# guxm2021/SVT_SpeechBrain

Hardware: AMD Instinct MI355X
Metric: 10s@16kHz clips/sec encoder+CTC forward, wav2vec2-base, 1/2/4/8 MI355X (higher is better)
Workload: dtype bf16; 1 GPU; wav2vec2-base audio-only AMT forward (encoder + 20-way head + frame decode), 32 x 10 s @16 kHz mono clips per GPU; global_batch=32, per_gpu_batch=32, samples_per_clip=160000, frames_per_clip=499, parallelism=clips sharded over 1 rank(s), streams=2, inputs=resident in HBM

## Files before the change

svt_speechbrain_amd/csrc/gemm_dma.hip:

```cpp
#include "common.h"
#include <map>
#include <mutex>
#include <utility>

namespace svt {
namespace {

__device__ __forceinline__ float gelu_erf(float x) { return gelu_fast(x); }
__device__ __forceinline__ float apply_act(float v, int act) {
  if (act == ACT_GELU) return gelu_erf(v);
  if (act == ACT_RELU) return v > 0.f ? v : 0.f;
  return v;
}

typedef const void __attribute__((address_space(1)))* gptr_t;
typedef void __attribute__((address_space(3)))* lptr_t;

template <int N> __device__ __forceinline__ void wait_vm() { asm volatile("s_waitcnt vmcnt(%0)" ::"n"(N) : "memory"); }

struct BiasRegs { float v[8]; };
template <bool OUT32>
__device__ __forceinline__ BiasRegs load_bias_regs(const GemmArgs& p, const float* bias, int lane, int wn, int n0) {
  BiasRegs b;
#pragma unroll
// ... 881 lines not shown
      long long* o = p.trace + 65536 + ((long)blockIdx.x * 8 + wave) * 32;
#pragma unroll
      for (int i = 0; i < 5; ++i) o[i] = sst[i];
      o[9] = nk; o[10] = gs; o[11] = STQ;
    }
  }
#undef X3S_S
#undef X3S_COMMIT
#undef X3S_LOAD
#undef X3S_MMA
#undef X3S_VARS
#undef X3S_END
  wait_vm<0>();
  __syncthreads();
  const float* bias = p.bias ? p.bias + (long)z2 * p.bias_z2 : nullptr;
  float* patch = (float*)lds + wave * (16 * 68);
  if constexpr (DBG == 3) {
#pragma unroll
    for (int i = 0; i < NB; ++i) asm volatile("" ::"v"(acc[i][0]), "v"(acc[i][1]));
    return;
  }
#pragma unroll
  for (int g = 0; g < NBS; ++g) {
    const BiasRegs br = load_bias_regs<true>(p, bias, lane, g, n0);
    epilogue_block<2, 64, true>(p, acc[4 * g][0], acc[4 * g + 1][0], acc[4 * g + 2][0], acc[4 * g + 3][0], 0, patch, lane, wave, g, m0, n0, czoff, br);
    epilogue_block<2, 64, true>(p, acc[4 * g][1], acc[4 * g + 1][1], acc[4 * g + 2][1], acc[4 * g + 3][1], 1, patch, lane, wave, g, m0, n0, czoff, br);
  }
}

template <bool F16>
__global__ void split_pack_kernel(const float* __restrict__ w, long n_rows, int K, unsigned short* __restrict__ out) {
  const long i = (long)blockIdx.x * blockDim.x + threadIdx.x;
  const long per_row = K / 8;
  if (i >= n_rows * per_row) return;
  const long n = i / per_row;
  const int k0 = (int)(i % per_row) * 8;
  const float* src = w + n * K + k0;
  unsigned short h[8], l[8];
#pragma unroll
  for (int j = 0; j < 8; ++j) {
    const float x = src[j];
    if constexpr (F16) {
      const _Float16 a = (_Float16)x, b = (_Float16)(x - (float)a);
      h[j] = __builtin_bit_cast(unsigned short, a);
      l[j] = __builtin_bit_cast(unsigned short, b);
    } else {
      const bf16_t a = (bf16_t)x, b = (bf16_t)(x - (float)a);
      h[j] = __builtin_bit_cast(unsigned short, a);
      l[j] = __builtin_bit_cast(unsigned short, b);
    }
  }
  unsigned short* dst = out + n * (2L * K) + (long)(k0 / 32) * 64 + (k0 % 32);
#pragma unroll
  for (int j = 0; j < 8; ++j) { dst[j] = h[j]; dst[32 + j] = l[j]; }
}

template <int BM>
int launch_pers(const GemmArgs& a, hipStream_t s) {
  const int tiles_m = (a.M + BM - 1) / BM, tiles_n = (a.N + 255) / 256;
  const int ntiles = tiles_m * tiles_n;
  int nblk = ntiles < 256 ? ((ntiles + 7) / 8) * 8 : 256;
  const size_t lds_bytes = 5 * 32768;
  if (int r_ = ensure_dyn_lds((const void*)gemm_pers_kernel<BM>, (int)lds_bytes)) return r_;
  const double flops = 2.0 * a.M * (double)a.N * a.K;
  const double bytes = ((double)a.M * a.K + (double)a.N * a.K) * 2 + (double)a.M * a.N * (a.out_f32 ? 4 : 2);
  prof_begin(s);
  hipLaunchKernelGGL((gemm_pers_kernel<BM>), dim3(nblk), dim3(512), lds_bytes, s, a, tiles_n, ntiles);
  prof_end(s, flops, bytes, 0);
  SVT_LAUNCH_CHECK();
  return 0;
}

template <int BM, bool GEN = false, int NBW = 4>
int launch_pp8(const GemmArgs& a, hipStream_t s) {
  const int tiles_m = (a.M + BM - 1) / BM, tiles_n = (a.N + 64 * NBW - 1) / (64 * NBW);
  dim3 grid(tiles_m * tiles_n, a.nz, 1);
  const size_t lds_bytes = 5 * 32768;
  if (int r_ = ensure_dyn_lds((const void*)gemm_pp8_kernel<BM, GEN, NBW>, (int)lds_bytes)) return r_;
  const double flops = 2.0 * a.M * (double)a.N * a.K * a.nz;
  const double bytes = ((double)a.M * a.K + (double)a.N * a.K) * 2 * a.nz + (double)a.M * a.N * a.nz * (a.out_f32 ? 4 : 2);
  prof_begin(s);
  hipLaunchKernelGGL((gemm_pp8_kernel<BM, GEN, NBW>), grid, dim3(512), lds_bytes, s, a);
  prof_end(s, flops, bytes, 0);
  SVT_LAUNCH_CHECK();
  return 0;
}

}

namespace {
struct SplitW { void* packed; int N, K, kind; };
std::map<const void*, SplitW> g_split_w;
std::mutex g_split_mu;
}

int split_weights_register(const void* w_f32, long n_rows, int K, int kind, hipStream_t s) {
  if (kind != 2 && kind != 3) return 0;
  if (K % 32 || n_rows < 1) return 0;
  void* packed = nullptr;
  {
    std::lock_guard<std::mutex> lk(g_split_mu);
    auto it = g_split_w.find(w_f32);
    if (it != g_split_w.end() && it->second.N == (int)n_rows && it->second.K == K) packed = it->second.packed;
  }
  const bool reused = packed != nullptr;
  if (reused) SVT_HIP(hipDeviceSynchronize());
  if (!reused)
    if (int r = dev_alloc(&packed, (size_t)n_rows * K * 4)) return r;
  const long pieces = n_rows * (K / 8);
  if (kind == 3) hipLaunchKernelGGL((split_pack_kernel<true>), dim3((unsigned)((pieces + 255) / 256)), dim3(256), 0, s, (const float*)w_f32, n_rows, K, (unsigned short*)packed);
  else hipLaunchKernelGGL((split_pack_kernel<false>), dim3((unsigned)((pieces + 255) / 256)), dim3(256), 0, s, (const float*)w_f32, n_rows, K, (unsigned short*)packed);
  SVT_LAUNCH_CHECK();
  std::lock_guard<std::mutex> lk(g_split_mu);
  auto it = g_split_w.find(w_f32);
  if (it != g_split_w.end() && !reused) dev_free(it->second.packed);
  g_split_w[w_f32] = SplitW{packed, (int)n_rows, K, kind};
  return 0;
}
void split_weights_forget(const void* w_f32) {
  std::lock_guard<std::mutex> lk(g_split_mu);
  auto it = g_split_w.find(w_f32);
  if (it == g_split_w.end()) return;
  dev_free(it->second.packed);
  g_split_w.erase(it);
}
int g_gemm_walk = -1;
int g_conv_kperm = 1;
int g_gemm_persist_wgs = 256;
int gemm_walk_pm(const GemmArgs& a, int bm) {
  if (g_gemm_walk >= 0) return g_gemm_walk;
  const int tiles_n = a.N / 256, tiles_m = (a.M + bm - 1) / bm;
  const double w_bytes = (double)a.N * a.K * 2.0;
  if (tiles_n < 8 || tiles_m < 16 || w_bytes <= 4.0 * 1024 * 1024) return 0;
  return 8;
}
int g_x3_pairs = 1;
int launch_gemm_x3(int kind, const GemmArgs& a, hipStream_t s) {
  if (a.a_pairs) {
    if (!gemm_x3q_eligible(a) || a.ldw != a.K) { set_error("gemm: pair-row operand outside the contract of gemm_x3q_kernel"); return -1; }
    const void* packed = nullptr;
    {
      std::lock_guard<std::mutex> lk(g_split_mu);
      auto it = g_split_w.upper_bound(a.W);
      if (it != g_split_w.begin()) {
        --it;
        const size_t off = (const char*)a.W - (const char*)it->first;
        if (it->second.kind == kind && it->second.K == a.K && off % ((size_t)a.K * 4) == 0 && off / ((size_t)a.K * 4) + a.N <= (size_t)it->second.N)
          packed = (const char*)it->second.packed + off;
      }
    }
    if (!packed) { set_error("gemm: pair-row product against a weight matrix that was not registered as split"); return -1; }
    const int cands[3] = {256, 192, 128};
    const int slab_cost[3] = {167, 137, 105};
    long best_cost = -1;
    int best = 256;
    for (int i = 0; i < 3; ++i) {
      const long blocks = (long)((a.M + cands[i] - 1) / cands[i]) * (a.N / 256);
      const long cost = ((blocks + 255) / 256) * slab_cost[i];
      if (best_cost < 0 || cost < best_cost) { best_cost = cost; best = cands[i]; }
    }
    if (g_gemm_force_bm == 256 || g_gemm_force_bm == 192 || g_gemm_force_bm == 128) best = g_gemm_force_bm;
    GemmArgs g = a;
    g.planes_f16 = kind == 3;
    const double flops = 2.0 * a.M * (double)a.N * a.K;
    const double bytes = ((double)a.M * a.K + (double)a.N * a.K + (double)a.M * a.N) * 4;
    prof_begin(s);
    if (g_gemm_p1x && g.K >= 96) { if (int r_ = launch_gemm_p1x(kind, g, packed, best, s)) return r_; }
    else if (int r_ = launch_gemm_x3q(kind, g, packed, best, s)) return r_;
    prof_end(s, flops, bytes, 0);
    return 0;
  }
  const bool batched = a.nz > 1;
  if (a.gen || a.nz < 1 || a.K % 32 || a.N < 128 || a.M < 128 || !a.c_vec || a.ldw != a.K || a.alpha != 1.f || (a.a_rstride & 3) ||
      (a.a_bstride & 3) || ((uintptr_t)a.A & 15))
    return 1;
  if (!batched && (a.w_z1 || a.w_z2 || a.a_z1 || a.a_z2 || a.c_z1 || a.c_z2)) return 1;
  if (batched && (a.planes || a.resid || a.nz2 < 1 || a.nz % a.nz2 || (a.a_z1 & 3) || (a.a_z2 & 3) || (a.c_z1 & 3) || (a.c_z2 & 3) || (a.bias_z2 & 3) ||
                  a.w_z1 % a.K || a.w_z2 % a.K || a.nz > 65535))
    return 1;
  const void* packed = nullptr;
  {
    std::lock_guard<std::mutex> lk(g_split_mu);
    auto it = g_split_w.upper_bound(a.W);
    if (it == g_split_w.begin()) return 1;
    --it;
    const char* base = (const char*)it->first;
    const size_t off = (const char*)a.W - base;
    if (it->second.kind != kind || it->second.K != a.K || off % ((size_t)a.K * 4) != 0) return 1;
    const size_t row = off / ((size_t)a.K * 4);
    const size_t last_z_row = batched ? ((size_t)(a.nz / a.nz2 - 1) * a.w_z1 + (size_t)(a.nz2 - 1) * a.w_z2) / (size_t)a.K : 0;
    if (row + last_z_row + a.N > (size_t)it->second.N) return 1;
    packed = (const char*)it->second.packed + row * (size_t)a.K * 4;
  }
  {
    const unsigned long clips = 255 / (unsigned long)(a.a_rpb > 0 ? a.a_rpb : 1) + 1;
    const unsigned long bs = (unsigned long)(a.a_bstride > 0 ? a.a_bstride : 0), rs = (unsigned long)(a.a_rstride > 0 ? a.a_rstride : 0);
    if (a.a_bstride < 0 || a.a_rstride <= 0 || (clips * bs + 256ul * rs + (unsigned long)a.K) * 4 >= 0xF0000000ul ||
        (unsigned long)a.N * a.K * 4 >= 0xF0000000ul)
      return 1;
  }
  const size_t lds_bytes = 5 * 32768;
  GemmArgs g = a;
  g.out_f32 = 1;
  g.planes_f16 = kind == 3;
  if (g_gemm_dbg == 9 && a.resid) {
    g.trace = (long long*)a.resid;
    g.resid = nullptr;
    g.stamp_ends = g_stamp_ends;
  }
  const double flops = 2.0 * a.M * (double)a.N * a.K * a.nz;
  const double bytes = ((double)a.M * a.K + (double)a.N * a.K + (double)a.M * a.N) * 4 * a.nz;
  const long tm = (a.M + 255) / 256;
  const long t256 = tm * ((a.N + 255) / 256), t192 = tm * ((a.N + 191) / 192);
  auto rounds = [](long t) { return (t + 255) / 256; };
  const bool narrow = a.N % 192 == 0 && rounds(t192) * 3 < rounds(t256) * 4;
  prof_begin(s);
  const bool x3p_ok = !batched && gemm_x3p_eligible(g) && g_gemm_variant != 30 && g_gemm_variant != 31 && g_gemm_variant != 32 && g_gemm_variant != 33;
  if (x3p_ok && (g_gemm_variant == 34 || (a.act == ACT_GELU && t256 > 256) || t256 >= 1024)) {
    g.dbg = g_gemm_dbg == 9 ? 0 : g_gemm_dbg;
    if (int r_ = launch_gemm_x3p(kind, g, packed, s)) return r_;
#ifdef SVT_DIAG
  } else if (g.trace && kind == 3 && g.stamp_ends >= 1 && g.stamp_ends <= 4) {
#define SVT_X3S_STAMP(NBS_, D_)                                                                                    \
  {                                                                                                                 \
    if (int r_ = ensure_dyn_lds((const void*)gemm_x3s_kernel<true, NBS_, D_>, (int)lds_bytes)) return r_;           \
    hipLaunchKernelGGL((gemm_x3s_kernel<true, NBS_, D_>), dim3((unsigned)(narrow ? t192 : t256)), dim3(512), lds_bytes, s, g, packed); \
  }
    if (narrow) {
      if (g.stamp_ends == 1) SVT_X3S_STAMP(3, 11) else if (g.stamp_ends == 2) SVT_X3S_STAMP(3, 12)
      else if (g.stamp_ends == 3) SVT_X3S_STAMP(3, 13) else SVT_X3S_STAMP(3, 14)
    } else {
      if (g.stamp_ends == 1) SVT_X3S_STAMP(4, 11) else if (g.stamp_ends == 2) SVT_X3S_STAMP(4, 12)
      else if (g.stamp_ends == 3) SVT_X3S_STAMP(4, 13) else SVT_X3S_STAMP(4, 14)
    }
#undef SVT_X3S_STAMP
  } else if ((g_gemm_variant == 31 || g_gemm_variant == 33) && kind == 3) {
    if (g_gemm_variant == 31) {
      if (int r_ = ensure_dyn_lds((const void*)gemm_x3s_kernel<true, 4, 1>, (int)lds_bytes)) return r_;
      hipLaunchKernelGGL((gemm_x3s_kernel<true, 4, 1>), dim3((unsigned)t256), dim3(512), lds_bytes, s, g, packed);
    } else {
      if (int r_ = ensure_dyn_lds((const void*)gemm_x3s_kernel<true, 4, 3>, (int)lds_bytes)) return r_;
      hipLaunchKernelGGL((gemm_x3s_kernel<true, 4, 3>), dim3((unsigned)t256), dim3(512), lds_bytes, s, g, packed);
    }
#endif
  } else if (narrow) {
    if (kind == 3) {
      if (int r_ = ensure_dyn_lds((const void*)gemm_x3s_kernel<true, 3>, (int)lds_bytes)) return r_;
      hipLaunchKernelGGL((gemm_x3s_kernel<true, 3>), dim3((unsigned)t192, (unsigned)a.nz), dim3(512), lds_bytes, s, g, packed);
    } else {
      if (int r_ = ensure_dyn_lds((const void*)gemm_x3s_kernel<false, 3>, (int)lds_bytes)) return r_;
      hipLaunchKernelGGL((gemm_x3s_kernel<false, 3>), dim3((unsigned)t192, (unsigned)a.nz), dim3(512), lds_bytes, s, g, packed);
    }
  } else {
    if (kind == 3) {
      if (int r_ = ensure_dyn_lds((const void*)gemm_x3s_kernel<true, 4>, (int)lds_bytes)) return r_;
      hipLaunchKernelGGL((gemm_x3s_kernel<true, 4>), dim3((unsigned)t256, (unsigned)a.nz), dim3(512), lds_bytes, s, g, packed);
    } else {
      if (int r_ = ensure_dyn_lds((const void*)gemm_x3s_kernel<false, 4>, (int)lds_bytes)) return r_;
      hipLaunchKernelGGL((gemm_x3s_kernel<false, 4>), dim3((unsigned)t256, (unsigned)a.nz), dim3(512), lds_bytes, s, g, packed);
    }
  }
  prof_end(s, flops, bytes, 0);
  SVT_LAUNCH_CHECK();
  return 0;
}

bool gemm_dma_eligible(const GemmArgs& a) { return a.K % 64 == 0 && a.N >= 128 && a.M >= 128 && a.c_vec && a.N % 8 == 0; }

int g_gemm_dbg = 0;
int g_gemm_force_bm = 0;
int g_gemm_variant = 0;
int g_stamp_ends = 0;
int g_gemm_ring = 0;
int launch_gemm_dma(const GemmArgs& a0, hipStream_t s) {
  GemmArgs a = a0;
  a.dbg = g_gemm_dbg;
  if (a.dbg == 9) { a.trace = (long long*)a.resid; a.resid = nullptr; if (g_gemm_variant) a.dbg = g_gemm_variant; }
  const int tiles_n = (a.N + 255) / 256;
  const int cands[4] = {256, 192, 128, 64};
  const int slab_cost[4] = {167, 137, 105, 85};
  long best_cost = -1;
  int best = 256;
  for (int i = 0; i < 4; ++i) {
    const int bm = cands[i];
    const long blocks = (long)((a.M + bm - 1) / bm) * tiles_n * a.nz;
    const long rounds = (blocks + 255) / 256;
    const long cost = rounds * slab_cost[i];
    if (best_cost < 0 || cost < best_cost) { best_cost = cost; best = bm; }
  }
  if (g_gemm_force_bm) best = g_gemm_force_bm;
  if (a.gen) {
    if (a.N <= 128) return launch_pp8<256, true, 2>(a, s);
    if (best == 256) return launch_pp8<256, true>(a, s);
    if (best == 192) return launch_pp8<192, true>(a, s);
    return launch_pp8<128, true>(a, s);
  }
  const long ntiles = (long)((a.M + best - 1) / best) * tiles_n;
  if (g_gemm_variant >= 50 && g_gemm_variant < 80 && gemm_pps_eligible(a)) {
    GemmArgs b = a;
    b.dbg = g_gemm_variant % 10;
    return launch_gemm_pps(b, g_gemm_force_bm ? g_gemm_force_bm : (best < 128 ? 128 : best), s);
  }
  if (g_gemm_variant != 49 && g_gemm_ring == 0 && best >= 128 && ntiles >= 100 && gemm_pps_eligible(a)) {
    if (g_gemm_p1w && a.K >= 192 && (!a.trace || g_gemm_p1w == 2) && (g_gemm_p1w == 2 || !(a.act == ACT_GELU && a.K < 1024))) {
      if (a.W_kperm && g_conv_kperm && a.kperm_taps >= 2 && a.kperm_taps <= 3 && a.kperm_cin % 64 == 0 && a.K == a.kperm_taps * a.kperm_cin && a.ldw == a.K) {
        GemmArgs b = a;
        b.W = a.W_kperm; b.k_taps = a.kperm_taps; b.k_cin = a.kperm_cin;
        return launch_gemm_p1w(b, best, s);
      }
      return launch_gemm_p1w(a, best, s);
    }
    return launch_gemm_pps(a, best, s);
  }
  const bool pers_ok = !a.resid && a.nz == 1 && a.K >= 128 && a.N % 256 == 0 && a.c_z1 == 0 && a.c_z2 == 0 &&
                       a.a_z1 == 0 && a.a_z2 == 0 && a.w_z1 == 0 && a.w_z2 == 0;
  int mode = g_gemm_ring;
  if (mode == 0) mode = (pers_ok && ntiles >= 512) ? 4 : 2;
  if (mode == 4 && pers_ok) {
    if (best == 256) return launch_pers<256>(a, s);
    if (best == 192) return launch_pers<192>(a, s);
    if (best == 128) return launch_pers<128>(a, s);
    return launch_pers<64>(a, s);
  }
  if (best == 256) return launch_pp8<256>(a, s);
  if (best == 192) return launch_pp8<192>(a, s);
  if (best == 128) return launch_pp8<128>(a, s);
  return launch_pp8<64>(a, s);
}

}
```

svt_speechbrain_amd/csrc/gemm_p1w.hip:

```cpp
#include "common.h"

namespace svt {
namespace {

#ifndef SVT_P1W_STORE_AUX
#define SVT_P1W_STORE_AUX 16
#endif
template <int N> __device__ __forceinline__ void p1_wait_vm() { asm volatile("s_waitcnt vmcnt(%0)" ::"n"(N) : "memory"); }

__device__ __forceinline__ void p1_dma(unsigned voff, const void* sbase, unsigned lds_addr) {
  asm volatile("s_mov_b32 m0, %0\n\ts_nop 0\n\tglobal_load_lds_dwordx4 %1, %2" ::"s"(lds_addr), "v"(voff), "s"(sbase) : "memory");
}

typedef unsigned p1_u32x4 __attribute__((ext_vector_type(4)));

template <int BM, int ACT, bool TR = false>
__global__ __launch_bounds__(256) void gemm_p1w_kernel(GemmArgs p, int tiles_n, int ntiles) {
  constexpr int BN = 256, BK = 64, NSLOT = 5;
  constexpr int MB = BM / 32;
  constexpr int GA = BM / 32;
  constexpr int GW = BN / 32;
  constexpr int SLOT = 2048;
  constexpr int MPG = MB / 2;
  static_assert(MB == 8 || MB == 6 || MB == 4, "BM in {256, 192, 128}");
  extern __shared__ __attribute__((aligned(16))) uint4 lds[];

  const int tid = threadIdx.x, lane = tid & 63;
  const int wave = __builtin_amdgcn_readfirstlane(tid >> 6);
  const int wm = wave & 1, wn = wave >> 1;
  const int nblk = gridDim.x, b = blockIdx.x;
  const int per = nblk >> 3;
  const int lbase = (b & 7) * per + (b >> 3);
  if (lbase >= ntiles) return;
  const int my_tiles = (ntiles - lbase + nblk - 1) / nblk;
  const int tiles_m = ntiles / tiles_n;
  auto tile_col = [&](int logical) -> int { int tm, tn; tile_walk(logical, tiles_m, tiles_n, p.walk_pm, tm, tn); return tn; };

  const char* gA = (const char*)p.A;
  const char* gW = (const char*)p.W;
  const int r8 = lane >> 3, ch = (lane & 7) ^ r8;
  unsigned aofE[GA], aofO[GA];
  unsigned wofE, wofO;
  const long w_col = (long)p.ldw * 2;
  const bool plain_a = p.a_rpb >= p.M;
  auto setup = [&](int logical, unsigned (&ao)[GA], unsigned& wo) {
    int tile_n, tile_m;
    tile_walk(logical, tiles_m, tiles_n, p.walk_pm, tile_m, tile_n);
    const int m0 = tile_m * BM, n0 = tile_n * BN;
#pragma unroll
    for (int i = 0; i < GA; ++i) {
      int m = m0 + (wave + 4 * i) * 8 + r8;
      if (m > p.M - 1) m = p.M - 1;
      if (plain_a) ao[i] = (unsigned)(((long)m * p.a_rstride + ch * 8) * 2);
      else ao[i] = (unsigned)(((long)(m / p.a_rpb) * p.a_bstride + (long)(m % p.a_rpb) * p.a_rstride + ch * 8) * 2);
    }
    {
      const int rho = wave * 8 + r8;
      const int n = n0 + (rho & 15) * 8 + ((rho >> 4) & 7);
      wo = (unsigned)(((long)n * p.ldw + ch * 8) * 2);
    }
  };
  auto w_piece = [&](int i) -> long { return (long)(2 * (i & 3) + 128 * (i >> 2)) * w_col; };
  const unsigned lds0 = __builtin_amdgcn_readfirstlane((unsigned)(size_t)(void __attribute__((address_space(3)))*)lds);
  auto lds_unit = [&](int slot, int i) -> unsigned { return lds0 + (unsigned)(slot * SLOT + (wave + 4 * i) * 64) * 16u; };

  f32x4 acc[8][MB];
  const int cq = lane >> 4, r16 = lane & 15, rr8 = r16 & 7;
  const int frag0 = (r16 >> 3) * 64 + rr8 * 8 + (cq ^ rr8);
  const int frag1 = (r16 >> 3) * 64 + rr8 * 8 + ((4 + cq) ^ rr8);
  const int xoff = (wm * MB) * 128;
  const int woff = (wn * 8) * 128;

  const int nk = p.K / BK;
  const int taps = p.k_taps;
  auto aoff = [&](int kk) -> long {
    if (taps <= 1) return (long)kk * (BK * 2);
    const int cb = taps == 3 ? (kk * 21846) >> 16 : kk >> 1;
    return ((long)(kk - cb * taps) * p.k_cin + (long)cb * BK) * 2;
  };
  const bool no_epi = p.dbg == 3, has_bias = p.bias != nullptr;
  constexpr bool tr = TR;
  long long t_begin = 0, t_first = 0, t_epi = 0, c_first = 0, c_wait = 0;
  if (tr) t_begin = wall_clock64();
  setup(lbase, aofE, wofE);
  setup(my_tiles > 1 ? nblk + lbase : lbase, aofO, wofO);
  f32x4 bq[2];
#pragma unroll
  for (int j = 0; j < 2; ++j) bq[j] = f32x4{0.f, 0.f, 0.f, 0.f};
  if (has_bias) {
    const float* bp = p.bias + (tile_col(lbase) * BN + wn * 128 + (lane & 15) * 8);
    asm volatile("global_load_dwordx4 %0, %2, off\n\tglobal_load_dwordx4 %1, %2, off offset:16"
                 : "+v"(bq[0]), "+v"(bq[1]) : "v"(bp) : "memory");
  }
#pragma unroll
  for (int i = 0; i < GA; ++i) p1_dma(aofE[i], gA, lds_unit(0, i));
#pragma unroll
  for (int i = 0; i < GW; ++i) p1_dma(wofE, gW + w_piece(i), lds_unit(1, i));
#pragma unroll
  for (int i = 0; i < GA; ++i) p1_dma(aofE[i], gA + aoff(1), lds_unit(2, i));
#pragma unroll
  for (int i = 0; i < GW; ++i) p1_dma(wofE, gW + BK * 2 + w_piece(i), lds_unit(3, i));
  p1_wait_vm<GA + GW>();
  asm volatile("" : "+v"(bq[0]), "+v"(bq[1]));
  __builtin_amdgcn_s_barrier();
  if (tr) { t_first = wall_clock64(); c_first = __builtin_amdgcn_s_memtime(); }

  bf16x8 xf[2][MB], wf[8];
  int sa = 0, ti = 0;

  auto tile_end = [&]() {
    ++ti;
    if (ti + 1 < my_tiles) {
      unsigned na[GA], nw;
      setup((ti + 1) * nblk + lbase, na, nw);
      const bool into_odd = (ti & 1) == 0;
#pragma unroll
      for (int i = 0; i < GA; ++i) { aofO[i] = into_odd ? na[i] : aofO[i]; aofE[i] = into_odd ? aofE[i] : na[i]; }
      wofO = into_odd ? nw : wofO; wofE = into_odd ? wofE : nw;
    }
  };

  auto read_x = [&](int slot, int ks, int buf, int jj) {
    xf[buf][jj] = __builtin_bit_cast(bf16x8, lds[slot * SLOT + xoff + jj * 128 + (ks ? frag1 : frag0)]);
  };
  auto read_w = [&](int slot, int ks, int nb) {
    const int ws = slot + 1 >= NSLOT ? slot + 1 - NSLOT : slot + 1;
    wf[nb] = __builtin_bit_cast(bf16x8, lds[ws * SLOT + woff + nb * 128 + (ks ? frag1 : frag0)]);
  };

#pragma unroll
  for (int jj = 0; jj < MB; ++jj) read_x(0, 0, 0, jj);
#pragma unroll
  for (int nb = 0; nb < 8; ++nb) read_w(0, 0, nb);

  auto kstep = [&](auto buf_c, auto req_c, auto first_c, int rs, int rks, bool ev_a, const char* srcA, int slotA, bool ev_w, const char* srcW, int slotW) {
    constexpr int BUF = decltype(buf_c)::value, REQ = decltype(req_c)::value;
    constexpr bool FIRST = decltype(first_c)::value != 0;
#pragma unroll
    for (int i = 0; i < 16; ++i) {
      const int nb = i >> 1, mb0 = (i & 1) * MPG;
      if constexpr (FIRST) {
        const float bv = bq[nb >> 2][nb & 3];
        const f32x4 b4 = {bv, bv, bv, bv};
#pragma unroll
        for (int j = 0; j < MPG; ++j) acc[nb][mb0 + j] = SVT_MFMA_16x16x32(xf[BUF][mb0 + j], wf[nb], b4);
      } else {
#pragma unroll
        for (int j = 0; j < MPG; ++j) acc[nb][mb0 + j] = SVT_MFMA_16x16x32(xf[BUF][mb0 + j], wf[nb], acc[nb][mb0 + j]);
      }
      if (i & 1) read_w(rs, rks, nb);
      if (i < MB) read_x(rs, rks, BUF ^ 1, i);
      if (REQ == 1 && (i & 1) && (i >> 1) < GA) p1_dma(ev_a ? aofE[i >> 1] : aofO[i >> 1], srcA, lds_unit(slotA, i >> 1));
      if (REQ == 2 && (i & 1) && (i >> 1) < GW) p1_dma(ev_w ? wofE : wofO, srcW + w_piece(i >> 1), lds_unit(slotW, i >> 1));
      __builtin_amdgcn_sched_barrier(0);
    }
  };
  constexpr bool FIN_VGPR = !(BM == 256 && ACT == ACT_GELU);
  constexpr int NREQ = (GW + GA + MB - 1) / MB;
  constexpr int LAST_W_BLOCK = (GW - 1) / NREQ;
  constexpr int STORES_AFTER_W = (MB - LAST_W_BLOCK) * 4;
  static_assert(NREQ * MB >= GW + GA, "the last k-step issues every request of the next tile's head");
  static_assert(GA + STORES_AFTER_W <= 63 && GA + GW <= 63, "vmcnt holds 6 bits");
  auto kstep_last = [&](int rs, bool ev, const char* srcA, int slotA, const char* srcW, int slotW) {
    const int logical = ti * nblk + lbase;
    int tile_n, tile_m;
    tile_walk(logical, tiles_m, tiles_n, p.walk_pm, tile_m, tile_n);
    const int m0 = tile_m * BM, n0 = tile_n * BN;
    const long rows_left = (long)p.M - m0;
    const unsigned long nbytes = (unsigned long)rows_left * p.ldc * 2;
    const unsigned nrec = nbytes > 0xFFFFFFF0ul ? 0xFFFFFFF0u : (unsigned)nbytes;
    char* cbase = (char*)p.C + (long)m0 * p.ldc * 2;
    const auto crsrc = __builtin_amdgcn_make_buffer_rsrc(cbase, 0, nrec, 0x00020000);
    const unsigned off0 = (unsigned)((((long)(wm * (BM / 2) + 4 * (lane >> 4))) * p.ldc + n0 + wn * 128 + (lane & 15) * 8) * 2);
    const unsigned row_pitch = (unsigned)(p.ldc * 2);
#pragma unroll
    for (int mb = 0; mb < MB; ++mb) {
      f32x4 fin[8];
      if constexpr (FIN_VGPR) {
#pragma unroll
        for (int nb = 0; nb < 8; ++nb) fin[nb] = SVT_MFMA_16x16x32(xf[1][mb], wf[nb], acc[nb][mb]);
      } else {
#pragma unroll
        for (int nb = 0; nb < 8; ++nb) acc[nb][mb] = SVT_MFMA_16x16x32(xf[1][mb], wf[nb], acc[nb][mb]);
#pragma unroll
        for (int nb = 0; nb < 8; ++nb) asm volatile("" : "+a"(acc[nb][mb]));
      }
      read_x(rs, 0, 0, mb);
#pragma unroll
      for (int q = 0; q < NREQ; ++q) {
        const int rq = mb * NREQ + q;
        if (rq < GW) p1_dma(ev ? wofE : wofO, srcW + w_piece(rq), lds_unit(slotW, rq));
        else if (rq < GW + GA) p1_dma(ev ? aofE[rq - GW] : aofO[rq - GW], srcA, lds_unit(slotA, rq - GW));
      }
      __builtin_amdgcn_sched_barrier(0);
      if (!no_epi) {
#pragma unroll
        for (int r = 0; r < 4; ++r) {
          bf16x8 o;
          if constexpr (ACT == ACT_GELU) {
            f32x2_t g[4];
#pragma unroll
            for (int j = 0; j < 4; ++j) g[j] = FIN_VGPR ? f32x2_t{fin[2 * j][r], fin[2 * j + 1][r]} : f32x2_t{acc[2 * j][mb][r], acc[2 * j + 1][mb][r]};
            if constexpr (FIN_VGPR) {
              gelu_bf16x2_x4(g);
            } else {
#pragma unroll
              for (int j = 0; j < 4; ++j) { g[j] = gelu_bf16x2(g[j]); asm volatile("" : "+v"(g[j])); }
            }
#pragma unroll
            for (int j = 0; j < 4; ++j) {
              o[2 * j] = (bf16_t)g[j].x;
              o[2 * j + 1] = (bf16_t)g[j].y;
            }
          } else {
#pragma unroll
            for (int j = 0; j < 8; ++j) o[j] = (bf16_t)(FIN_VGPR ? fin[j][r] : acc[j][mb][r]);
          }
          __builtin_amdgcn_raw_buffer_store_b128(__builtin_bit_cast(p1_u32x4, o), crsrc, off0 + (mb * 16 + r) * row_pitch, 0, SVT_P1W_STORE_AUX);
          if constexpr (ACT == ACT_GELU) __builtin_amdgcn_sched_barrier(0);
        }
      } else {
#pragma unroll
        for (int nb = 0; nb < 8; ++nb) { if constexpr (FIN_VGPR) asm volatile("" ::"v"(fin[nb])); else asm volatile("" ::"a"(acc[nb][mb])); }
      }
      __builtin_amdgcn_sched_barrier(0);
    }
  };
  using c0 = std::integral_constant<int, 0>;
  using c1 = std::integral_constant<int, 1>;
  using c2 = std::integral_constant<int, 2>;
  auto slot_add = [](int s_, int d) { const int t = s_ + d; return t >= NSLOT ? t - NSLOT : t; };
  auto mid_barrier = [&](auto out_c) {
    long long c0_ = 0;
    if (tr) c0_ = __builtin_amdgcn_s_memtime();
    p1_wait_vm<decltype(out_c)::value>();
    asm volatile("s_waitcnt lgkmcnt(0)" ::: "memory");
    __builtin_amdgcn_sched_barrier(0);
    __builtin_amdgcn_s_barrier();
    if (tr) c_wait += __builtin_amdgcn_s_memtime() - c0_;
  };
  using w_a = std::integral_constant<int, GA>;
  using w_as = std::integral_constant<int, GA + STORES_AFTER_W>;

  for (int t = 0; t < my_tiles; ++t) {
    const bool te = (ti & 1) == 0;
    const bool first_tile = t == 0;
    asm volatile("" : "+v"(bq[0]), "+v"(bq[1]));
    {
      const char* sA = gA + aoff(2);
      const char* sW = gW + 2L * (BK * 2);
      if (first_tile) {
        kstep(c0{}, c1{}, c1{}, sa, 1, te, sA, slot_add(sa, 4), te, sW, sa);
        mid_barrier(w_a{});
      } else {
        kstep(c0{}, c0{}, c1{}, sa, 1, te, sA, slot_add(sa, 4), te, sW, sa);
        if (no_epi) mid_barrier(w_a{}); else mid_barrier(w_as{});
      }
      kstep(c1{}, c2{}, c0{}, slot_add(sa, 2), 0, te, sA, 0, te, sW, sa);
      sa = slot_add(sa, 2);
    }
    for (int k = 1; k + 1 < nk; ++k) {
      const bool cur2 = k + 2 < nk;
      const bool ev = cur2 == te;
      const int kk = cur2 ? k + 2 : k + 2 - nk;
      const long ko = (long)kk * (BK * 2), koa = aoff(kk);
      kstep(c0{}, c1{}, c0{}, sa, 1, ev, gA + koa, slot_add(sa, 4), ev, gW + ko, sa);
      mid_barrier(w_a{});
      kstep(c1{}, c2{}, c0{}, slot_add(sa, 2), 0, ev, gA + koa, 0, ev, gW + ko, sa);
      sa = slot_add(sa, 2);
    }
    {
      if (has_bias) {
        const float* bp = p.bias + (tile_col(ti + 1 < my_tiles ? (ti + 1) * nblk + lbase : lbase) * BN + wn * 128 + (lane & 15) * 8);
        asm volatile("global_load_dwordx4 %0, %2, off\n\tglobal_load_dwordx4 %1, %2, off offset:16"
                     : "+v"(bq[0]), "+v"(bq[1]) : "v"(bp) : "memory");
      }
      const bool ev = !te;
      kstep(c0{}, c1{}, c0{}, sa, 1, ev, gA + aoff(1), slot_add(sa, 4), ev, gW, sa);
      mid_barrier(w_a{});
      long long t_e0 = 0;
      if (tr) t_e0 = wall_clock64();
      kstep_last(slot_add(sa, 2), ev, gA + aoff(2), slot_add(sa, 1), gW + 1L * (BK * 2), sa);
      sa = slot_add(sa, 2);
#pragma unroll
      for (int nb = 0; nb < 8; ++nb) read_w(sa, 0, nb);
      if (tr) t_epi += wall_clock64() - t_e0;
    }
    tile_end();
  }
  long long t_loop = 0;
  if (tr) t_loop = wall_clock64();
  p1_wait_vm<0>();
  if (tr && lane == 0) {
    if ((wave & 1) == 0) {
      long long* o = p.trace + ((long)blockIdx.x * 2 + (wave >> 1)) * 8;
      o[0] = t_begin; o[1] = t_first; o[2] = t_loop - t_first - t_epi; o[3] = t_epi; o[4] = t_loop; o[5] = my_tiles;
      o[6] = __builtin_amdgcn_s_memtime() - c_first; o[7] = BM;
    }
    p.trace[524288 + (long)blockIdx.x * 4 + wave] = c_wait;
  }
}

template <int BM, int ACT, bool TR = false>
int launch_p1w_t(const GemmArgs& a, hipStream_t s) {
  const int tiles_m = (a.M + BM - 1) / BM, tiles_n = a.N / 256;
  const int ntiles = tiles_m * tiles_n;
  const int nblk = ntiles < g_gemm_persist_wgs ? ((ntiles + 7) / 8) * 8 : g_gemm_persist_wgs;
  const size_t lds_bytes = 5 * 32768;
  GemmArgs aw = a;
  aw.walk_pm = gemm_walk_pm(a, BM);
  if (int r_ = ensure_dyn_lds((const void*)gemm_p1w_kernel<BM, ACT, TR>, (int)lds_bytes)) return r_;
  const double flops = 2.0 * a.M * (double)a.N * a.K;
  const double bytes = ((double)a.M * a.K + (double)a.N * a.K) * 2 + (double)a.M * a.N * 2;
  prof_begin(s);
  hipLaunchKernelGGL((gemm_p1w_kernel<BM, ACT, TR>), dim3(nblk), dim3(256), lds_bytes, s, aw, tiles_n, ntiles);
  prof_end(s, flops, bytes, 0);
  SVT_LAUNCH_CHECK();
  return 0;
}

}

int g_gemm_p1w = 1;

int launch_gemm_p1w(const GemmArgs& a, int bm, hipStream_t s) {
#ifdef SVT_DIAG
  if (a.trace) {
    if (bm == 256) return launch_p1w_t<256, ACT_NONE, true>(a, s);
    return launch_p1w_t<192, ACT_NONE, true>(a, s);
  }
#else
  if (a.trace) { set_error("gemm_p1w: the stamped instantiations are built by `make DIAG=1` only"); return -1; }
#endif
  if (a.act == ACT_GELU) {
    if (bm == 256) return launch_p1w_t<256, ACT_GELU>(a, s);
    if (bm == 192) return launch_p1w_t<192, ACT_GELU>(a, s);
    return launch_p1w_t<128, ACT_GELU>(a, s);
  }
  if (bm == 256) return launch_p1w_t<256, ACT_NONE>(a, s);
  if (bm == 192) return launch_p1w_t<192, ACT_NONE>(a, s);
  return launch_p1w_t<128, ACT_NONE>(a, s);
}

}
```

Before: 6327 clips/s.

## Interleave next-row MFMAs with GELU epilogue in p1w GEMM and enable for all GELU

The final k-step of the p1w GEMM now software-pipelines the last MFMAs: the MFMAs for row block mb+1 are issued between the epilogue store rows of block mb, so matrix work overlaps the GELU and store instructions. The separate fin VGPR staging path is removed and GELU on BM=256 is split into two-wide chunks. The dispatcher also drops the exclusion that kept GELU GEMMs with K<1024 off the p1w kernel, so more layers use it. The no_epi debug flag is now honored only in the traced variant. The risks are extra register pressure and a slower p1w path on the smaller-K GELU GEMMs now routed to it.

```diff
diff --git a/svt_speechbrain_amd/csrc/gemm_dma.hip b/svt_speechbrain_amd/csrc/gemm_dma.hip
--- a/svt_speechbrain_amd/csrc/gemm_dma.hip
+++ b/svt_speechbrain_amd/csrc/gemm_dma.hip
@@ -1207,7 +1207,7 @@
     return launch_gemm_pps(b, g_gemm_force_bm ? g_gemm_force_bm : (best < 128 ? 128 : best), s);
   }
   if (g_gemm_variant != 49 && g_gemm_ring == 0 && best >= 128 && ntiles >= 100 && gemm_pps_eligible(a)) {
-    if (g_gemm_p1w && a.K >= 192 && (!a.trace || g_gemm_p1w == 2) && (g_gemm_p1w == 2 || !(a.act == ACT_GELU && a.K < 1024))) {
+    if (g_gemm_p1w && a.K >= 192 && (!a.trace || g_gemm_p1w == 2)) {
       if (a.W_kperm && g_conv_kperm && a.kperm_taps >= 2 && a.kperm_taps <= 3 && a.kperm_cin % 64 == 0 && a.K == a.kperm_taps * a.kperm_cin && a.ldw == a.K) {
         GemmArgs b = a;
         b.W = a.W_kperm; b.k_taps = a.kperm_taps; b.k_cin = a.kperm_cin;
diff --git a/svt_speechbrain_amd/csrc/gemm_p1w.hip b/svt_speechbrain_amd/csrc/gemm_p1w.hip
--- a/svt_speechbrain_amd/csrc/gemm_p1w.hip
+++ b/svt_speechbrain_amd/csrc/gemm_p1w.hip
@@ -78,7 +78,8 @@
     const int cb = taps == 3 ? (kk * 21846) >> 16 : kk >> 1;
     return ((long)(kk - cb * taps) * p.k_cin + (long)cb * BK) * 2;
   };
-  const bool no_epi = p.dbg == 3, has_bias = p.bias != nullptr;
+  const bool has_bias = p.bias != nullptr;
+  const bool no_epi = TR && p.dbg == 3;
   constexpr bool tr = TR;
   long long t_begin = 0, t_first = 0, t_epi = 0, c_first = 0, c_wait = 0;
   if (tr) t_begin = wall_clock64();
@@ -155,7 +156,6 @@
       __builtin_amdgcn_sched_barrier(0);
     }
   };
-  constexpr bool FIN_VGPR = !(BM == 256 && ACT == ACT_GELU);
   constexpr int NREQ = (GW + GA + MB - 1) / MB;
   constexpr int LAST_W_BLOCK = (GW - 1) / NREQ;
   constexpr int STORES_AFTER_W = (MB - LAST_W_BLOCK) * 4;
@@ -173,18 +173,39 @@
     const auto crsrc = __builtin_amdgcn_make_buffer_rsrc(cbase, 0, nrec, 0x00020000);
     const unsigned off0 = (unsigned)((((long)(wm * (BM / 2) + 4 * (lane >> 4))) * p.ldc + n0 + wn * 128 + (lane & 15) * 8) * 2);
     const unsigned row_pitch = (unsigned)(p.ldc * 2);
+    auto mfma = [&](int mb, int nb) { acc[nb][mb] = SVT_MFMA_16x16x32(xf[1][mb], wf[nb], acc[nb][mb]); };
+    auto epi_row = [&](int mb, int r) {
+      bf16x8 o;
+      if constexpr (ACT == ACT_GELU) {
+        f32x2_t g[4];
+#pragma unroll
+        for (int j = 0; j < 4; ++j) g[j] = f32x2_t{acc[2 * j][mb][r], acc[2 * j + 1][mb][r]};
+        if constexpr (BM != 256) {
+          gelu_bf16x2_x4(g);
+        } else {
+          f32x2_t h[2] = {g[0], g[1]};
+          gelu_bf16x2_xn<2>(h);
+          g[0] = h[0]; g[1] = h[1];
+          h[0] = g[2]; h[1] = g[3];
+          gelu_bf16x2_xn<2>(h);
+          g[2] = h[0]; g[3] = h[1];
+        }
+#pragma unroll
+        for (int j = 0; j < 4; ++j) {
+          o[2 * j] = (bf16_t)g[j].x;
+          o[2 * j + 1] = (bf16_t)g[j].y;
+        }
+      } else {
+#pragma unroll
+        for (int j = 0; j < 8; ++j) o[j] = (bf16_t)acc[j][mb][r];
+      }
+      __builtin_amdgcn_raw_buffer_store_b128(__builtin_bit_cast(p1_u32x4, o), crsrc, off0 + (mb * 16 + r) * row_pitch, 0, SVT_P1W_STORE_AUX);
+    };
+#pragma unroll
+    for (int nb = 0; nb < 8; ++nb) mfma(0, nb);
+    __builtin_amdgcn_sched_barrier(0);
 #pragma unroll
     for (int mb = 0; mb < MB; ++mb) {
-      f32x4 fin[8];
-      if constexpr (FIN_VGPR) {
-#pragma unroll
-        for (int nb = 0; nb < 8; ++nb) fin[nb] = SVT_MFMA_16x16x32(xf[1][mb], wf[nb], acc[nb][mb]);
-      } else {
-#pragma unroll
-        for (int nb = 0; nb < 8; ++nb) acc[nb][mb] = SVT_MFMA_16x16x32(xf[1][mb], wf[nb], acc[nb][mb]);
-#pragma unroll
-        for (int nb = 0; nb < 8; ++nb) asm volatile("" : "+a"(acc[nb][mb]));
-      }
       read_x(rs, 0, 0, mb);
 #pragma unroll
       for (int q = 0; q < NREQ; ++q) {
@@ -193,37 +214,13 @@
         else if (rq < GW + GA) p1_dma(ev ? aofE[rq - GW] : aofO[rq - GW], srcA, lds_unit(slotA, rq - GW));
       }
       __builtin_amdgcn_sched_barrier(0);
-      if (!no_epi) {
-#pragma unroll
-        for (int r = 0; r < 4; ++r) {
-          bf16x8 o;
-          if constexpr (ACT == ACT_GELU) {
-            f32x2_t g[4];
-#pragma unroll
-            for (int j = 0; j < 4; ++j) g[j] = FIN_VGPR ? f32x2_t{fin[2 * j][r], fin[2 * j + 1][r]} : f32x2_t{acc[2 * j][mb][r], acc[2 * j + 1][mb][r]};
-            if constexpr (FIN_VGPR) {
-              gelu_bf16x2_x4(g);
-            } else {
-#pragma unroll
-              for (int j = 0; j < 4; ++j) { g[j] = gelu_bf16x2(g[j]); asm volatile("" : "+v"(g[j])); }
-            }
-#pragma unroll
-            for (int j = 0; j < 4; ++j) {
-              o[2 * j] = (bf16_t)g[j].x;
-              o[2 * j + 1] = (bf16_t)g[j].y;
-            }
-          } else {
-#pragma unroll
-            for (int j = 0; j < 8; ++j) o[j] = (bf16_t)(FIN_VGPR ? fin[j][r] : acc[j][mb][r]);
-          }
-          __builtin_amdgcn_raw_buffer_store_b128(__builtin_bit_cast(p1_u32x4, o), crsrc, off0 + (mb * 16 + r) * row_pitch, 0, SVT_P1W_STORE_AUX);
-          if constexpr (ACT == ACT_GELU) __builtin_amdgcn_sched_barrier(0);
-        }
-      } else {
-#pragma unroll
-        for (int nb = 0; nb < 8; ++nb) { if constexpr (FIN_VGPR) asm volatile("" ::"v"(fin[nb])); else asm volatile("" ::"a"(acc[nb][mb])); }
-      }
-      __builtin_amdgcn_sched_barrier(0);
+#pragma unroll
+      for (int r = 0; r < 4; ++r) {
+        if (mb + 1 < MB) { mfma(mb + 1, 2 * r); mfma(mb + 1, 2 * r + 1); }
+        if (no_epi) asm volatile("" ::"a"(acc[2 * r][mb]), "a"(acc[2 * r + 1][mb]));
+        else epi_row(mb, r);
+        __builtin_amdgcn_sched_barrier(0);
+      }
     }
   };
   using c0 = std::integral_constant<int, 0>;
@@ -254,7 +251,7 @@
         mid_barrier(w_a{});
       } else {
         kstep(c0{}, c0{}, c1{}, sa, 1, te, sA, slot_add(sa, 4), te, sW, sa);
-        if (no_epi) mid_barrier(w_a{}); else mid_barrier(w_as{});
+        if (p.dbg == 3) mid_barrier(w_a{}); else mid_barrier(w_as{});
       }
       kstep(c1{}, c2{}, c0{}, slot_add(sa, 2), 0, te, sA, 0, te, sW, sa);
       sa = slot_add(sa, 2);
```

Result: no change. 6334 clips/s (median of 6 runs) (+0.1%).
